# themattinthehatt/behavenet

Measured on AMD Instinct MI355X. Metric: AE training frames/sec (128x128x1, batch 256), higher is better.
Workload: dtype f32; 1 GPU; configs[1]: conv AE default arch, 1x128x128 f32 frames resident in HBM, 12 latents, batch 256 (chunks 200+56), fwd+bwd+Adam(amsgrad)

## Files before the change

### behavenet_amd/_hip.py

```python

import ctypes
import os

import torch

_LIB_NAME = 'libbehavenet_hip.so'
_LIB_PATH = os.environ.get('BN_HIP_LIB') or os.path.join(
    os.path.dirname(os.path.abspath(__file__)), _LIB_NAME)
_lib = None

ACT_NONE, ACT_LRELU, ACT_SIGMOID = 0, 1, 2

PROF_NONE, PROF_CONV_FWD, PROF_CONV_BWD_D, PROF_CONV_BWD_W = 0, 1, 2, 3
PROF_CONVT_FWD, PROF_CONVT_BWD_D, PROF_CONVT_BWD_W, PROF_ADAM = 4, 5, 6, 7
PROF_LINEAR_FWD, PROF_LINEAR_BWD = 8, 9

_c_int, _c_float, _c_size_t, _c_void_p = ctypes.c_int, ctypes.c_float, ctypes.c_size_t, ctypes.c_void_p

_CONV_GEOM = [_c_int] * 12
_ACT_WS = [_c_int, _c_float, _c_void_p, _c_size_t, _c_void_p]

OP_CONV_FWD, OP_CONV_BWD_D, OP_CONV_BWD_W = 1, 2, 3
OP_CONVT_FWD, OP_CONVT_BWD_D, OP_CONVT_BWD_W = 4, 5, 6

SIGNATURES = {
    'bn_version': (_c_int, []),
    'bn_build_arch': (ctypes.c_char_p, []),
    'bn_error_string': (ctypes.c_char_p, [_c_int]),
    'bn_set_force_generic': (_c_int, [_c_int]),
    'bn_set_bigk1_block_bytes': (_c_size_t, [_c_size_t]),
    'bn_conv_ws_bytes': (_c_size_t, [_c_int] + _CONV_GEOM),
    'bn_conv_taps_bytes': (_c_size_t, [_c_int] + _CONV_GEOM),
    'bn_conv_taps_pad': (_c_int, [_c_int, _c_void_p, _c_void_p, _c_void_p, _c_void_p]),
    'bn_conv2d_fwd': (_c_int, [_c_void_p] * 5 + _CONV_GEOM + _ACT_WS),
    'bn_conv2d_fwd_u8_ws_bytes': (_c_size_t, _CONV_GEOM + [_c_int]),
    'bn_conv2d_fwd_u8': (_c_int, [_c_void_p] * 4 + _CONV_GEOM + _ACT_WS),
    'bn_conv2d_bwd_data': (_c_int, [_c_void_p] * 5 + _CONV_GEOM + _ACT_WS),
    'bn_conv2d_bwd_weight': (
        _c_int, [_c_void_p] * 4 + _CONV_GEOM + [_c_int, _c_void_p, _c_size_t, _c_void_p]),
    'bn_convT2d_fwd': (_c_int, [_c_void_p] * 5 + _CONV_GEOM + _ACT_WS),
    'bn_convT2d_bwd_data': (_c_int, [_c_void_p] * 5 + _CONV_GEOM + _ACT_WS),
    'bn_convT2d_bwd_weight': (
        _c_int, [_c_void_p] * 4 + _CONV_GEOM + [_c_int, _c_void_p, _c_size_t, _c_void_p]),
    'bn_batchnorm_ws_bytes': (_c_size_t, [_c_int, _c_int]),
    'bn_batchnorm_stats': (_c_int, [_c_void_p] * 3 + [_c_int] * 3 + [_c_void_p, _c_size_t, _c_void_p]),
    'bn_batchnorm_finalize': (_c_int, [_c_void_p] * 5 + [_c_int] + [_c_float] * 3 + [_c_void_p]),
    'bn_batchnorm_act_fwd': (_c_int, [_c_void_p] * 6 + [_c_int] * 4 + [_c_float, _c_void_p]),
    'bn_batchnorm_train_fwd_chunks': (
        _c_int, [_c_void_p] * 11 + [_c_int] * 3 + [_c_float, _c_int, _c_float, _c_void_p, _c_size_t,
                                                  _c_void_p]),
    'bn_batchnorm_act_bwd_chunks': (
        _c_int, [_c_void_p] * 10 + [_c_int, _c_void_p] + [_c_int] * 4 + [_c_float, _c_void_p, _c_size_t,
                                                                        _c_void_p]),
    'bn_batchnorm_act_bwd': (
        _c_int, [_c_void_p] * 9 + [_c_int] * 6 + [_c_float, _c_void_p, _c_size_t, _c_void_p]),
    'bn_batchnorm_moment': (_c_int, [_c_void_p] * 3 + [_c_int] * 3 + [_c_void_p, _c_size_t, _c_void_p]),
    'bn_batchnorm_bwd_reduce': (
        _c_int, [_c_void_p] * 7 + [_c_int] * 4 + [_c_float, _c_void_p, _c_size_t, _c_void_p]),
    'bn_batchnorm_bwd_apply': (
        _c_int, [_c_void_p] * 9 + [_c_int] * 3 + [_c_float, _c_int, _c_float, _c_void_p]),
    'bn_maxpool2d_fwd': (_c_int, [_c_void_p] * 3 + [_c_int] * 9 + [_c_void_p]),
    'bn_maxpool2d_bwd': (_c_int, [_c_void_p] * 3 + [_c_int] * 9 + [_c_void_p]),
    'bn_maxpool2d_act_fwd': (_c_int, [_c_void_p] * 3 + [_c_int] * 4 + [ctypes.c_float, _c_void_p]),
    'bn_conv2d_pool2_act_fwd': (_c_int, [_c_void_p] * 5 + _CONV_GEOM + [_c_int, _c_float, _c_void_p]),
    'bn_conv2d_pool2_act_ok': (_c_int, _CONV_GEOM),
    'bn_conv2d_pool2_bwd_weight_ws_bytes': (_c_size_t, _CONV_GEOM),
# ... 237 lines not shown
    _check(load().bn_convT2d_fwd(
        _ptr(x, 'x'), _ptr(w, 'w'), _ptr(w5, 'w5', allow_none=True), _ptr(b, 'b', allow_none=True), _ptr(y, 'y'),
        *geom, act, slope, ws, nb, _stream()), 'bn_convT2d_fwd')
    return y


def convT2d_bwd_data(dy, w, geom, dact_src, dact, slope, w5=None):
    N, Ci, Hi, Wi = geom[:4]
    dx = torch.empty((N, Ci, Hi, Wi), dtype=torch.float32, device=dy.device)
    ws, nb = _workspace(OP_CONVT_BWD_D, geom, dy.device)
    _check(load().bn_convT2d_bwd_data(
        _ptr(dy, 'dy'), _ptr(w, 'w'), _ptr(w5, 'w5', allow_none=True), _ptr(dx, 'dx'),
        _ptr(dact_src, 'dact_src', allow_none=True), *geom, dact, slope, ws, nb, _stream()), 'bn_convT2d_bwd_data')
    return dx


def convT2d_bwd_weight(x, dy, dw, db, geom, accumulate):
    ws, nb = _workspace(OP_CONVT_BWD_W, geom, x.device)
    _check(lib_call('bn_convT2d_bwd_weight')(
        _ptr(x, 'x'), _ptr(dy, 'dy'), _ptr(dw, 'dw'), _ptr(db, 'db', allow_none=True), *geom,
        int(accumulate), ws, nb, _stream()), 'bn_convT2d_bwd_weight')


def conv2d_bf16_ok(geom, first=False):
    lib = load()
    return bool((lib.bn_conv2d_first_bf16_ok if first else lib.bn_conv2d_bf16_ok)(*[int(v) for v in geom]))


def conv_pack_w_bf16_bytes(w_shape):
    K, C, R, S = [int(v) for v in w_shape]
    return int(load().bn_conv_pack_w_bf16_bytes(K, C, R, S))


def conv_pack_w_bf16(w, out):
    K, C, R, S = w.shape
    if out.numel() * out.element_size() < conv_pack_w_bf16_bytes(w.shape):
        raise HipLibraryError('conv_pack_w_bf16: output buffer too small')
    _check(load().bn_conv_pack_w_bf16(_ptr(w, 'w'), out.data_ptr(), K, C, R, S, _stream()),
           'bn_conv_pack_w_bf16')
    return out


def _bf16_out(out, shape, dtype, device, what):
    if out is None:
        return torch.empty(shape, dtype=dtype, device=device)
    if tuple(out.shape) != tuple(shape) or out.dtype != dtype:
# ... 730 lines not shown
```

### behavenet_amd/csrc/bn_fast.h

```cpp
#pragma once
#include "bn_common.h"

struct BnFastPlan {
    bool supported;
    const char* kernel_name;
    size_t ws_bytes;
    int variant;
    int a, b, c, d;
};

BnFastPlan bn_fast_down_plan(const BnGeom& g);
BnFastPlan bn_fast_up_plan(const BnGeom& g);
BnFastPlan bn_fast_wgrad_plan(const BnGeom& g);

int bn_launch_down_fast(const BnFastPlan& plan, const float* big, const float* w,
                        const float* bias, float* out, const float* dact_src, const BnGeom& g,
                        int act, int dact, float slope, void* ws, hipStream_t st);
int bn_launch_up_fast(const BnFastPlan& plan, const float* small, const float* w,
                      const float* bias, float* out, const float* dact_src, const BnGeom& g,
                      int act, int dact, float slope, void* ws, hipStream_t st);
int bn_launch_wgrad_fast(const BnFastPlan& plan, const float* small, const float* big, float* dw,
                         const BnGeom& g, int accumulate, void* ws, hipStream_t st,
                         float* db = nullptr, int bias_side = 0, bool* bias_done = nullptr);

bool bn_wgrad_pool_c1_ok(const BnGeom& g);
size_t bn_wgrad_pool_c1_ws_bytes(const BnGeom& g);
int bn_launch_wgrad_pool_c1(const float* x, const float* dy, const float* y, const int* idx, float* dw, float* db,
                            const BnGeom& g, int act, float slope, int accumulate, void* ws, hipStream_t st);
bool bn_s1in1_pool_ok(const BnGeom& g);
int bn_launch_s1in1_pool(const float* big, const float* w, const float* bias, float* y, int* idx, const BnGeom& g,
                         int act, float slope, hipStream_t st);
bool bn_down2_pool_ok(const BnGeom& g);
int bn_launch_down2_pool(const float* big, const float* w, const float* bias, float* y, int* idx, const BnGeom& g,
                         int act, float slope, hipStream_t st);
bool bn_down2_supported(const BnGeom& g, int MR, int NR);
bool bn_down2_m16_supported(const BnGeom& g, int NR);
int bn_down2_splits(const BnGeom& g, int MR, int NR);
float bn_down2_fill(const BnGeom& g, int MR, int NR);
int bn_launch_down2(int MR, int NR, const float* big, const float* w, const float* bias,
                    float* out, const float* dact_src, const BnGeom& g, int act, int dact,
                    float slope, hipStream_t st, int splits = 1, void* ws = nullptr);

BnFastPlan bn_wgrad4_plan(const BnGeom& g);
int bn_launch_wgrad4(const BnFastPlan& plan, const float* small, const float* big, float* dw,
                     const BnGeom& g, int accumulate, void* ws, hipStream_t st, float* db,
                     int bias_side, bool* bias_done);

BnFastPlan bn_s5_up_plan(const BnGeom& g);
BnFastPlan bn_s5_wgrad_plan(const BnGeom& g);
int bn_launch_up_s5(const float* small, const float* w, const float* bias, float* out,
                    const float* dact_src, const BnGeom& g, int act, int dact, float slope,
                    hipStream_t st);
int bn_launch_wgrad_s5(const float* small, const float* big, float* dw, const BnGeom& g,
                       int accumulate, hipStream_t st);

BnFastPlan bn_edge_wgrad_plan(const BnGeom& g);
int bn_launch_edge_wgrad(const BnFastPlan& plan, const float* small, const float* big, float* dw,
                         const BnGeom& g, int accumulate, void* ws, hipStream_t st,
                         float* db = nullptr, int bias_side = 0, bool* bias_done = nullptr);
bool bn_s1c1_ok(const BnGeom& g);
int bn_launch_s1c1(const float* big, const float* w, const float* bias, float* out, const float* dact_src,
                   const BnGeom& g, int act, int dact, float slope, hipStream_t st);
bool bn_s1in1_ok(const BnGeom& g);
int bn_launch_s1in1(const float* big, const float* w, const float* bias, float* out, const float* dact_src,
                    const BnGeom& g, int act, int dact, float slope, hipStream_t st);
BnFastPlan bn_edge_down_plan(const BnGeom& g);
const char* bn_edge_down_kernel_name(const BnGeom& g, int act, bool has_dact, bool u8);
const char* bn_edge_up_kernel_name(const BnGeom& g, bool loss);
int bn_launch_edge_down(const float* big, const float* w, const float* bias, float* out,
// ... 43 lines not shown
```

### behavenet_amd/csrc/capi.hip

```cpp
#include <math.h>
#include <stdio.h>
#include <stdlib.h>
#include <string.h>
#include <hip/hip_ext.h>
#include "bn_common.h"
#include "bn_launch.h"
#include "bn_fast.h"

namespace {
struct ProfState {
    int family = BN_PROF_NONE;
    int C = 0, K = 0;
    static const int kMaxSlots = 2048;
    hipEvent_t ev[4 * kMaxSlots];
    bool taken[kMaxSlots], bracketed[kMaxSlots];
    int created = 0;
    int used = 0;
    double total_ms = 0.0, main_ms = 0.0;
    long launches = 0, main_launches = 0;
    bool bracket = true;
    int nth = -1, seen = 0;
    char kernel_name[96] = "";
} g_prof;

// ... 1246 lines not shown
    const BnGeom g = convT_geom(N, Ci, Hi, Wi, Co, R, S, stride, crop_t, crop_l, Ho, Wo);
    if (!bn_geom_ok(g)) return BN_E_BADARG;
    return run_down(BN_PROF_CONVT_BWD_D, dy, w, w5, nullptr, dx, dact_src, g, BN_ACT_NONE, dact, slope,
                    ws, ws_bytes, (hipStream_t)stream);
}

extern "C" int bn_convT2d_bwd_weight(const float* x, const float* dy, float* dw, float* db, int N,
                                     int Ci, int Hi, int Wi, int Co, int R, int S, int stride,
                                     int crop_t, int crop_l, int Ho, int Wo, int accumulate,
                                     void* ws, size_t ws_bytes, bn_stream_t stream) {
    if (!x || !dy || !dw) return BN_E_BADARG;
    const BnGeom g = convT_geom(N, Ci, Hi, Wi, Co, R, S, stride, crop_t, crop_l, Ho, Wo);
    if (!bn_geom_ok(g)) return BN_E_BADARG;
    hipStream_t st = (hipStream_t)stream;
    bool bias_done = false;
    int rc = run_wgrad(BN_PROF_CONVT_BWD_W, x, dy, dw, g, accumulate, ws, ws_bytes, st, db, 2,
                       &bias_done);
    if (rc) return rc;
    if (db && !bias_done)
        rc = bn_launch_channel_sum(dy, db, N, Co, Ho * Wo, accumulate, ws, ws_bytes, st);
    return rc;
}

extern "C" int bn_act_fwd(const float* x, float* y, size_t n, int act, float slope,
                          bn_stream_t stream) {
    if (!x || !y || n == 0) return BN_E_BADARG;
    return bn_launch_act_fwd(x, y, n, act, slope, (hipStream_t)stream);
}

extern "C" int bn_act_bwd(const float* dy, const float* y, float* dpre, size_t n, int act,
                          float slope, bn_stream_t stream) {
    if (!dy || !y || !dpre) return BN_E_BADARG;
    if (n == 0) return 0;
    return bn_launch_act_bwd(dy, y, dpre, n, act, slope, (hipStream_t)stream);
}

extern "C" size_t bn_batchnorm_ws_bytes(int N, int C) {
    return (N > 0 && C > 0) ? bn_batchnorm_ws_bytes_impl(N, C) : 0;
}

extern "C" int bn_batchnorm_stats(const float* x, float* mean, float* var, int N, int C, int HW,
                                  void* ws, size_t ws_bytes, bn_stream_t stream) {
    if (!x || !mean || !var || N <= 0 || C <= 0 || HW <= 0) return BN_E_BADARG;
    if (!ws || ws_bytes < bn_batchnorm_ws_bytes_impl(N, C)) return BN_E_WORKSPACE;
    return bn_launch_bn_stats(x, mean, var, N, C, HW, ws, (hipStream_t)stream);
}
// ... 498 lines not shown
```

### behavenet_amd/csrc/conv_mfma_wgrad4.hip

```cpp
#include <stdlib.h>
#include "bn_common.h"
#include "bn_fast.h"
#include "bn_reduce.h"

typedef float floatx4 __attribute__((ext_vector_type(4)));
typedef float floatx2 __attribute__((ext_vector_type(2)));

#define W4_STR2(x) #x
#define W4_STR(x) W4_STR2(x)
#ifndef W4_LOOP_SHIFT
#define W4_LOOP_SHIFT 0
#endif
#define W4_THREADS 512
#define W4_TA 64
#define W4_TB 32
#define W4_TPX 64
#define W4_X0 4
#define W4_SLICES 8
#define W4_MAX_LDS (160 * 1024)
#define W4_OOB 0x7fffffff

static inline int ilog2_exact_w4(int v) {
    int l = 0;
    while ((1 << l) < v) ++l;
// ... 155 lines not shown
    }
}

template <int Q_, int ST_ = 2, int PTH_ = 0>
struct W4S {
    static constexpr int Q = Q_, ST = ST_, PT_H = PTH_ ? PTH_ : W4_TPX / Q, IH = ST * (PT_H - 1) + 5;
    static constexpr int KS = PT_H * Q / 4;
    static constexpr int RW = ST * Q + 8, C4 = RW / 4;
    static constexpr int ROWG = IH * C4;
    static constexpr int GPB = (ROWG & 1) ? ROWG : ROWG + 1;
    static constexpr int BCH = 4 * GPB;
    static constexpr int BIGG = W4_TB * GPB;
    static constexpr int SMALLW = W4_TA * W4_TPX;
    static constexpr int BUFW = SMALLW + 4 * ((BIGG + 63) / 64 * 64);
    static constexpr int NBIG = (BIGG + W4_THREADS - 1) / W4_THREADS;
    static constexpr int NSM = SMALLW / 4 / W4_THREADS;
};

__device__ __forceinline__ void w4_dma16(__amdgpu_buffer_rsrc_t rsrc, float* lds, int voffset,
                                         int soffset) {
    __builtin_amdgcn_raw_ptr_buffer_load_lds(rsrc, lds, 16, voffset, soffset, 0, 0);
}

template <int QQ, int BIAS, bool GEN, int KV, int ST = 2, int PTH = 0, bool CW = false, int NA = 4, int NB = 2>
__global__ __launch_bounds__(W4_THREADS, 1) void k_wgrad4s_mfma(
    const float* __restrict__ small, const float* __restrict__ big, float* __restrict__ part,
    float* __restrict__ bias_part, BnGeom g, int n_stages, int splits, int lg_tpf, int nbias, int ncb) {
    extern __shared__ __attribute__((aligned(16))) float smem[];
    using T = W4S<QQ, ST, PTH>;
    static_assert(ST == 2 || GEN, "stride 1: the general row limits");
    static_assert(!CW || (GEN && ST == 2 && (QQ & 3) == 0), "column windows: general stride-2 stages");
    constexpr int Q = T::Q, RW = T::RW, BUFW = T::BUFW;
    constexpr bool HALF = (Q & 3) == 2;
    static_assert(((Q & 3) == 0 || (HALF && ST == 2 && GEN && (T::PT_H & 1) == 0)) && T::KS >= 1 && T::KS <= 16,
                  "stage geometry");
    const int tid = threadIdx.x, lane = tid & 63;
    const int wv = __builtin_amdgcn_readfirstlane(tid >> 6);
    constexpr int NG = 8 / (NA * NB), KSG = T::KS / NG;
    static_assert(NA * NB * NG == 8 && KSG * NG == T::KS && KSG >= 1 && NG <= 4, "wave groups");
    static_assert(NG == 1 || (!HALF && !CW && (KSG & (KSG - 1)) == 0 &&
                              ((4 * KSG) % Q == 0 || Q % (4 * KSG) == 0)), "wave groups: whole rows or parts of one");
    const int blk = wv % (NA * NB), grp = wv / (NA * NB);
    const int ablk = NG == 1 ? wv >> 1 : blk / NB, bblk = NG == 1 ? wv & 1 : blk % NB;
    const int lj = lane & 15, kk = lane >> 4;

    const int n_btiles = (g.Cb + W4_TB - 1) / W4_TB;
    const int atile = blockIdx.x / n_btiles, btile = blockIdx.x - atile * n_btiles;
    const int a0 = atile * W4_TA, b0 = btile * W4_TB;
    const int PQ = g.Hs * g.Ws, HWb = g.Hb * g.Wb;

    floatx4 acc[25];
#pragma unroll
    for (int tp = 0; tp < 25; ++tp) acc[tp] = (floatx4){0.f, 0.f, 0.f, 0.f};
    float bsum = 0.f;

    const __amdgpu_buffer_rsrc_t rs_small = __builtin_amdgcn_make_buffer_rsrc(
        (void*)small, 0, (int)((size_t)g.N * g.Cs * PQ * 4), 0x00020000);
    const int pt_rows = ST == 2 ? 1 : g.pt;
    const int lead = pt_rows * g.Wb + (CW ? W4_X0 : 0);
    const __amdgpu_buffer_rsrc_t rs_big = __builtin_amdgcn_make_buffer_rsrc(
        (void*)(big - lead), 0, (int)(((size_t)g.N * g.Cb * HWb + lead) * 4), 0x00020000);
    int soff[T::NSM], srow = 0;
#pragma unroll
    for (int j = 0; j < T::NSM; ++j) {
        const int e = tid + W4_THREADS * j;
        const int a = e >> 4;
        const int pix0 = 4 * ((e & 15) ^ (a & 15));
        const int spix = CW ? (pix0 / Q) * g.Ws + (pix0 - (pix0 / Q) * Q) : pix0;
        soff[j] = (a0 + a < g.Cs && pix0 < 4 * T::KS) ? ((a0 + a) * PQ + spix) * 4 : W4_OOB;
        srow |= (pix0 / Q) << (8 * j);
// ... 117 lines not shown
                    }
                } else if (NG == 1) {
                    if (r == 3 && sx == 4 && ks < NDMA) {
                        if (more) issue_dma(ks, nbuf, n0n, p0n);
                    }
                } else if (sx == 4 && r < NG && ks * NG + r < NDMA) {
                    if (more) issue_dma(ks * NG + r, nbuf, n0n, p0n);
                }
                __builtin_amdgcn_sched_barrier(0);
            }
        }
    };

    const int tpf_mask = (1 << lg_tpf) - 1;
    const int tpf_gen = (g.Hs + T::PT_H - 1) / T::PT_H;
    auto frame_of = [&](const int s) __attribute__((always_inline)) {
        if constexpr (GEN) return lg_tpf == 0 ? s : (int)__umulhi((unsigned)s, (unsigned)lg_tpf);
        else return s >> lg_tpf;
    };
    auto row_of = [&](const int s, const int f) __attribute__((always_inline)) {
        if constexpr (GEN) return (s - f * tpf_gen) * T::PT_H;
        else return (s & tpf_mask) * T::PT_H;
    };
    int st = blockIdx.y;
    if (st < n_stages) {
        const int f0 = frame_of(st);
#pragma unroll
        for (int d = 0; d < NDMA; ++d) issue_dma(d, 0, f0, row_of(st, f0));
    }
    int ab_cur = abase[0], ab_oth = abase[1], bb_cur = bbase[0], bb_oth = bbase[1];
    int cur = 0;
#ifdef W4_LOOP_ALIGN
    asm volatile(".p2align " W4_STR(W4_LOOP_ALIGN) "\n .rept " W4_STR(W4_LOOP_SHIFT) "\n s_nop 0\n .endr" ::: "memory");
#endif
    for (; st < n_stages; st += splits) {
        asm volatile("s_waitcnt vmcnt(0)" ::: "memory");
        __syncthreads();
        const int nx = st + splits;
        const int fx = frame_of(nx);
        stage_body(ab_cur, bb_cur, bsp_cur, cur ^ 1, nx < n_stages, fx, row_of(nx, fx));
        cur ^= 1;
        int tmp = ab_cur; ab_cur = ab_oth; ab_oth = tmp;
        tmp = bb_cur; bb_cur = bb_oth; bb_oth = tmp;
        if (HALF) { tmp = bsp_cur; bsp_cur = bsp_oth; bsp_oth = tmp; }
    }

    if (BIAS != 0) {
        bsum += __shfl_xor(bsum, 16, 64);
        bsum += __shfl_xor(bsum, 32, 64);
        float* bdst = bias_part + ((size_t)blockIdx.y * NG + grp) * nbias;
        if (BIAS == 1 && btile == 0 && bblk == 0 && kk == 0) {
            const int a = a0 + ablk * 16 + lj;
            if (a < g.Cs) bdst[a] = bsum;
        }
        if (BIAS == 2 && atile == 0 && ablk == 0 && kk == 0) {
            const int bb = b0 + bblk * 16 + lj;
            if (bb < g.Cb) bdst[bb] = bsum;
        }
    }

    float* dst = part + ((size_t)blockIdx.y * NG + grp) * 25 * g.Cs * g.Cb;
    const int b = b0 + bblk * 16 + lj;
    if (b < g.Cb) {
#pragma unroll
        for (int tp = 0; tp < 25; ++tp) {
#pragma unroll
            for (int e = 0; e < 4; ++e) {
                const int a = a0 + ablk * 16 + 4 * kk + e;
                if (a < g.Cs) dst[((size_t)tp * g.Cs + a) * g.Cb + b] = acc[tp][e];
            }
        }
    }
}

static bool wgrad4_tile(const BnGeom& g, Wgrad4Tile* t, size_t* lds_bytes) {
    const int lgQ = ilog2_exact_w4(g.Ws), lgP = ilog2_exact_w4(g.Hs);
    if (lgQ < 2 || lgQ > 5 || lgP < 0) return false;
    if (g.pt != 1 || g.pl != 1) return false;
    if ((g.Wb & 3) != 0 || g.Wb < 2 * g.Ws) return false;
    const int PQ = g.Hs * g.Ws;
    if (PQ >= W4_TPX) {
        t->F = 1;
        t->PT_H = W4_TPX / g.Ws;
    } else {
        t->F = W4_TPX / PQ;
        t->PT_H = g.Hs;
    }
    t->lgPTQ = ilog2_exact_w4(t->PT_H * g.Ws);
    t->tiles_per_frame = (t->F == 1) ? g.Hs / t->PT_H : 1;
    t->n_stages = ((g.N + t->F - 1) / t->F) * t->tiles_per_frame;
    t->IH = 2 * (t->PT_H - 1) + 5;
    const int RW = 2 * g.Ws + 8;
    t->FSb = t->IH * RW;
    t->rows_per_b = t->F * t->IH;
    t->row_groups = t->rows_per_b * (RW / 4);
// ... 306 lines not shown
                                                    t.n_stages, t.splits, lg_tpf, t.nbias);
        W4S_CASE(3, 0) W4S_CASE(3, 1) W4S_CASE(3, 2) W4S_CASE(4, 0) W4S_CASE(4, 1) W4S_CASE(4, 2)
        W4S_CASE(5, 0) W4S_CASE(5, 1) W4S_CASE(5, 2)
#undef W4S_CASE
        }
    } else
    switch (ilog2_exact_w4(g.Ws)) {
        case 2: rc = launch_wgrad4<2>(grid, lds, st, small, big, (float*)ws, bias_part, g, t); break;
        case 3: rc = launch_wgrad4<3>(grid, lds, st, small, big, (float*)ws, bias_part, g, t); break;
        case 4: rc = launch_wgrad4<4>(grid, lds, st, small, big, (float*)ws, bias_part, g, t); break;
        case 5: rc = launch_wgrad4<5>(grid, lds, st, small, big, (float*)ws, bias_part, g, t); break;
        default: break;
    }
    if (rc) return rc;
    if (fuse) {
        rc = bn_launch_sum_partials_pair((const float*)ws, dw, 25 * g.Cs * g.Cb, g.Cs * g.Cb, 25,
                                         bias_part, db, t.nbias, t.splits, accumulate, st);
        if (bias_done) *bias_done = true;
        return rc;
    }
    return bn_launch_sum_partials((const float*)ws, dw, 25 * g.Cs * g.Cb, t.splits, accumulate,
                                  g.Cs * g.Cb, 25, st);
}
```

### behavenet_amd/hip_functions.py

```python

import collections.abc
import contextlib
import os
import threading
import warnings

import torch

from behavenet_amd import _hip

LRELU_SLOPE = 0.05

_direct_grads = False


class accumulate_into_param_grads(object):

    def __enter__(self):
        global _direct_grads
        self._prev = _direct_grads
        _direct_grads = True

    def __exit__(self, *exc):
        global _direct_grads
# ... 43 lines not shown
    o = _ones_cache.get(key)
    if o is None:
        o = torch.ones_like(t.detach())
        _ones_cache[key] = o
    return o


def backward_chunks(chunk_losses, streams=None, single_pass=False):
    global _single_pass, _use_side_stream
    _single_pass = bool(single_pass and len(chunk_losses) == 1)
    saved_side = _use_side_stream
    if _single_pass:
        _use_side_stream = False
    try:
        with accumulate_into_param_grads():
            for i, loss in enumerate(chunk_losses):
                stream = streams[i] if streams is not None and i < len(streams) else None
                seed = _ones_like(loss) if loss.dim() > 0 else None
                if stream is not None:
                    with torch.cuda.stream(stream):
                        loss.backward(seed)
                else:
                    loss.backward(seed)
    finally:
        _single_pass = False
        _use_side_stream = saved_side


_capturing = False


def capturing():
    return _capturing


class DeferredLoss(object):

    def __init__(self, tensors, fn, reduce_over_ranks=False):
        self.tensors, self.fn = tensors, fn
        self.reduce_over_ranks = bool(reduce_over_ranks)


class LazyLoss(collections.abc.Mapping):

    def __init__(self, readbacks, fn):
        self._rbs, self._fn, self._dict = readbacks, fn, None

    def resolve(self):
        if self._dict is None:
# ... 303 lines not shown
    taps = getattr(ctx, 'taps', None)
    for i in range(n_layers - 1, -1, -1):
        layer = plan[i]
        g = layer.geom(n)
        w = weights[i]
        x_in = acts[i]
        if x_in.dtype == torch.uint8:
            x_in = _hip.u8_to_unit_float(x_in) \
                if ctx.needs_input_grad[first_param + 2 * i] else None
        need_w = ctx.needs_input_grad[first_param + 2 * i]
        need_b = ctx.needs_input_grad[first_param + 1 + 2 * i]
        if need_w:
            gw = _grad_buffer(ctx.param_refs[2 * i])
            gb = _grad_buffer(ctx.param_refs[2 * i + 1]) if need_b else None
            direct = gw is not None and (gb is not None or not need_b)
            if direct:
                dw, db = gw, gb
            else:
                dw = torch.empty_like(w)
                db = torch.empty((layer.cout,), dtype=w.dtype, device=w.device) if need_b \
                    else None
            wgrad = _hip.conv2d_bwd_weight if layer.kind == 'conv' else _hip.convT2d_bwd_weight
            side = _side_stream(w.device) if (direct and _use_side_stream) else None
            if side is not None:
                main = torch.cuda.current_stream(w.device)
                ev = torch.cuda.Event()
                ev.record(main)
                with torch.cuda.stream(side):
                    side.wait_event(ev)
                    wgrad(x_in, dpre, dw, db, g, True)
                dpre.record_stream(side)
                x_in.record_stream(side)
                _report_ready(ctx.param_refs[2 * i:2 * i + 2])
            else:
                wgrad(x_in, dpre, dw, db, g, direct)
                if direct:
                    _report_ready(ctx.param_refs[2 * i:2 * i + 2])
            if not direct:
                grads[2 * i], grads[2 * i + 1] = dw, db
        if i > 0 or ctx.need_dx:
            dact_src = acts[i] if i > 0 else None
            dact = plan[i - 1].act if i > 0 else _hip.ACT_NONE
            w5 = taps[i] if taps else None
            if layer.kind == 'conv':
                dpre = _hip.conv2d_bwd_data(dpre, w, g, dact_src, dact, LRELU_SLOPE, w5=w5)
            else:
                dpre = _hip.convT2d_bwd_data(dpre, w, g, dact_src, dact, LRELU_SLOPE, w5=w5)
# ... 1035 lines not shown
```

### include/behavenet_hip.h

```cpp
#ifndef BEHAVENET_HIP_H
#define BEHAVENET_HIP_H

#include <stddef.h>

#ifdef __cplusplus
extern "C" {
#endif

#define BN_E_BADARG   (-1)
#define BN_E_SHAPE    (-2)
#define BN_E_WORKSPACE (-3)

#define BN_ACT_NONE    0
#define BN_ACT_LRELU   1
#define BN_ACT_SIGMOID 2

typedef void* bn_stream_t;

int         bn_version(void);
const char* bn_build_arch(void);
const char* bn_error_string(int code);

#define BN_OP_CONV_FWD    1
#define BN_OP_CONV_BWD_D  2
// ... 18 lines not shown
                       int N, int C, int H, int W, int K, int R, int S, int stride,
                       int pad_t, int pad_l, int P, int Q,
                       int dact, float slope, void* ws, size_t ws_bytes, bn_stream_t stream);

int bn_conv2d_bwd_weight(const float* x, const float* dy, float* dw, float* db,
                         int N, int C, int H, int W, int K, int R, int S, int stride,
                         int pad_t, int pad_l, int P, int Q,
                         int accumulate, void* ws, size_t ws_bytes, bn_stream_t stream);

int bn_convT2d_fwd(const float* x, const float* w, const float* w5, const float* b, float* y,
                   int N, int Ci, int Hi, int Wi, int Co, int R, int S, int stride,
                   int crop_t, int crop_l, int Ho, int Wo,
                   int act, float slope, void* ws, size_t ws_bytes, bn_stream_t stream);

int bn_convT2d_bwd_data(const float* dy, const float* w, const float* w5, float* dx, const float* dact_src,
                        int N, int Ci, int Hi, int Wi, int Co, int R, int S, int stride,
                        int crop_t, int crop_l, int Ho, int Wo,
                        int dact, float slope, void* ws, size_t ws_bytes, bn_stream_t stream);

int bn_convT2d_bwd_weight(const float* x, const float* dy, float* dw, float* db,
                          int N, int Ci, int Hi, int Wi, int Co, int R, int S, int stride,
                          int crop_t, int crop_l, int Ho, int Wo,
                          int accumulate, void* ws, size_t ws_bytes, bn_stream_t stream);

int bn_act_fwd(const float* x, float* y, size_t n, int act, float slope, bn_stream_t stream);
int bn_act_bwd(const float* dy, const float* y, float* dpre, size_t n,
               int act, float slope, bn_stream_t stream);

int bn_maxpool2d_fwd(const float* x, float* y, int* idx, int planes, int H, int W, int Ho, int Wo,
                     int k, int stride, int pad_t, int pad_l, bn_stream_t stream);
int bn_maxpool2d_bwd(const float* dy, const int* idx, float* dx, int planes, int H, int W,
                     int Ho, int Wo, int k, int stride, int pad_t, int pad_l, bn_stream_t stream);
int bn_conv2d_pool2_act_fwd(const float* x, const float* w, const float* b, float* y, int* idx,
                            int N, int C, int H, int W, int K, int R, int S, int stride,
                            int pad_t, int pad_l, int P, int Q, int act, float slope, bn_stream_t stream);
int bn_conv2d_pool2_act_ok(int N, int C, int H, int W, int K, int R, int S, int stride,
                           int pad_t, int pad_l, int P, int Q);
size_t bn_conv2d_pool2_bwd_weight_ws_bytes(int N, int C, int H, int W, int K, int R, int S, int stride,
                                           int pad_t, int pad_l, int P, int Q);
int bn_conv2d_pool2_bwd_weight(const float* x, const float* dy, const float* y, const int* idx, float* dw, float* db,
                               int N, int C, int H, int W, int K, int R, int S, int stride,
                               int pad_t, int pad_l, int P, int Q, int act, float slope, int accumulate,
                               void* ws, size_t ws_bytes, bn_stream_t stream);
int bn_maxpool2d_act_fwd(const float* x, float* y, int* idx, int planes, int H, int W, int act, float slope,
                         bn_stream_t stream);
int bn_maxpool2d_act_bwd(const float* dy, const float* y, const int* idx, float* dx, int planes, int H, int W,
// ... 188 lines not shown
```

Measured before the change: 58860 frames/s.

## Batch several small-layer weight-gradient convolutions into one persistent stream-K style launch

Weight-gradient work for eligible stride-2 5x5 layers is queued during the single-pass backward instead of being launched per layer. Up to eight such layers then run in one kernel that splits their tile×stage work evenly across all compute units into per-tile partial slabs, followed by one combine kernel that reduces the slabs into dw/db. This targets per-layer launch overhead and poor CU fill for small layers. The cost is extra workspace and a second reduction pass, and the gradients are now produced later, which delays when the parameters are reported ready for the optimizer.

```diff
diff --git a/behavenet_amd/_hip.py b/behavenet_amd/_hip.py
--- a/behavenet_amd/_hip.py
+++ b/behavenet_amd/_hip.py
@@ -42,6 +42,11 @@
     'bn_convT2d_bwd_data': (_c_int, [_c_void_p] * 5 + _CONV_GEOM + _ACT_WS),
     'bn_convT2d_bwd_weight': (
         _c_int, [_c_void_p] * 4 + _CONV_GEOM + [_c_int, _c_void_p, _c_size_t, _c_void_p]),
+    'bn_wgrad_jobs_ok': (_c_int, [_c_int] + _CONV_GEOM),
+    'bn_wgrad_jobs_ws_bytes': (_c_size_t, [_c_int, _c_void_p, _c_int]),
+    'bn_wgrad_jobs_plan': (_c_int, [_c_int, _c_void_p, _c_int, _c_void_p, _c_int]),
+    'bn_wgrad_jobs': (
+        _c_int, [_c_int] + [_c_void_p] * 6 + [_c_void_p, _c_size_t, _c_int, _c_void_p]),
     'bn_batchnorm_ws_bytes': (_c_size_t, [_c_int, _c_int]),
     'bn_batchnorm_stats': (_c_int, [_c_void_p] * 3 + [_c_int] * 3 + [_c_void_p, _c_size_t, _c_void_p]),
     'bn_batchnorm_finalize': (_c_int, [_c_void_p] * 5 + [_c_int] + [_c_float] * 3 + [_c_void_p]),
@@ -325,6 +330,61 @@
         int(accumulate), ws, nb, _stream()), 'bn_convT2d_bwd_weight')
 
 
+WGRAD_JOBS_MAX = 8
+_jobs_ok = {}
+
+
+def wgrad_jobs_ok(op, geom):
+    key = (_generic_epoch, op) + tuple(geom)
+    v = _jobs_ok.get(key)
+    if v is None:
+        v = _jobs_ok[key] = bool(load().bn_wgrad_jobs_ok(op, *[int(q) for q in geom]))
+    return v
+
+
+def _jobs_geoms(jobs):
+    flat = []
+    for op, geom in jobs:
+        flat.append(int(op))
+        flat.extend(int(v) for v in geom)
+    return (ctypes.c_int * (13 * len(jobs)))(*flat)
+
+
+def wgrad_jobs_ws_bytes(jobs, n_wg=0):
+    return int(load().bn_wgrad_jobs_ws_bytes(len(jobs), _jobs_geoms(jobs), int(n_wg)))
+
+
+def wgrad_jobs_plan(jobs, n_wg):
+    lib, geoms = load(), _jobs_geoms(jobs)
+    n = lib.bn_wgrad_jobs_plan(len(jobs), geoms, int(n_wg), None, 0)
+    _check(min(n, 0), 'bn_wgrad_jobs_plan')
+    segs = (ctypes.c_int * (6 * max(n, 1)))()
+    _check(min(lib.bn_wgrad_jobs_plan(len(jobs), geoms, int(n_wg), segs, n), 0), 'bn_wgrad_jobs_plan')
+    return [tuple(segs[6 * i:6 * i + 6]) for i in range(n)]
+
+
+def wgrad_jobs(jobs, n_wg=0, ws=None):
+    n = len(jobs)
+    if n == 0:
+        return
+    geoms = _jobs_geoms([(j[0], j[1]) for j in jobs])
+    lib = load()
+    if ws is None:
+        nbytes = int(lib.bn_wgrad_jobs_ws_bytes(n, geoms, int(n_wg)))
+        if nbytes == 0:
+            raise HipLibraryError('wgrad_jobs: a layer that bn_wgrad_jobs does not serve')
+        wsp = _arena(jobs[0][2].device, nbytes, 'wgrad_jobs')
+    else:
+        wsp, nbytes = ws.data_ptr(), ws.numel()
+    vp = ctypes.c_void_p * n
+    xp = vp(*[_ptr(j[2], 'x') for j in jobs])
+    dyp = vp(*[_ptr(j[3], 'dy') for j in jobs])
+    dwp = vp(*[_ptr(j[4], 'dw') for j in jobs])
+    dbp = vp(*[_ptr(j[5], 'db', allow_none=True) for j in jobs])
+    acc = (ctypes.c_int * n)(*[int(bool(j[6])) for j in jobs])
+    _check(lib.bn_wgrad_jobs(n, geoms, xp, dyp, dwp, dbp, acc, wsp, nbytes, int(n_wg), _stream()), 'bn_wgrad_jobs')
+
+
 def conv2d_bf16_ok(geom, first=False):
     lib = load()
     return bool((lib.bn_conv2d_first_bf16_ok if first else lib.bn_conv2d_bf16_ok)(*[int(v) for v in geom]))
diff --git a/behavenet_amd/csrc/bn_fast.h b/behavenet_amd/csrc/bn_fast.h
--- a/behavenet_amd/csrc/bn_fast.h
+++ b/behavenet_amd/csrc/bn_fast.h
@@ -45,6 +45,15 @@
 int bn_launch_wgrad4(const BnFastPlan& plan, const float* small, const float* big, float* dw,
                      const BnGeom& g, int accumulate, void* ws, hipStream_t st, float* db,
                      int bias_side, bool* bias_done);
+
+#define BN_WGRAD_JOBS_MAX 8
+#define BN_WGRAD_JOBS_MAX_TILES 16
+bool bn_wgrad4_jobs_geom_ok(const BnGeom& g, int bias_side);
+size_t bn_wgrad4_jobs_ws_bytes(int n_jobs, const BnGeom* gs, const int* bias, int n_wg);
+int bn_wgrad4_jobs_plan(int n_jobs, const BnGeom* gs, const int* bias, int n_wg, int* segs, int max_segs);
+int bn_launch_wgrad4_jobs(int n_jobs, const BnGeom* gs, const int* bias, const float* const* small,
+                          const float* const* big, float* const* dw, float* const* db, const int* accumulate,
+                          void* ws, size_t ws_bytes, int n_wg, hipStream_t st);
 
 BnFastPlan bn_s5_up_plan(const BnGeom& g);
 BnFastPlan bn_s5_wgrad_plan(const BnGeom& g);
diff --git a/behavenet_amd/csrc/capi.hip b/behavenet_amd/csrc/capi.hip
--- a/behavenet_amd/csrc/capi.hip
+++ b/behavenet_amd/csrc/capi.hip
@@ -1292,6 +1292,95 @@
     return rc;
 }
 
+static bool wgrad_jobs_route(const BnGeom& g, int bias_side) {
+    if (force_generic()) return false;
+    BnGeom g5;
+    BigK bk;
+    BigK1 b1;
+    if (taps_plan(2, g, &g5) || bigk_plan(2, g, &g5, &bk) || bigk1_plan(2, g, &g5, &b1) || chan_plan(2, g, &g5))
+        return false;
+    if (bn_qg2_wgrad_supported(g) || bn_qgemm_supported(g) || bn_s5win_supported(g) || s5_wgrad_by_col(g)) return false;
+    if (bn_s5_wgrad_plan(g).supported || bn_edge_wgrad_plan(g).supported) return false;
+    const BnFastPlan plan = bn_fast_wgrad_plan(g);
+    return plan.supported && plan.variant == 4 && bn_wgrad4_jobs_geom_ok(g, bias_side);
+}
+static bool wgrad_jobs_geom(const int* q, BnGeom* g, int* side) {
+    if (q[0] == BN_OP_CONV_BWD_W) {
+        *g = conv_geom(q[1], q[2], q[3], q[4], q[5], q[6], q[7], q[8], q[9], q[10], q[11], q[12]);
+        *side = 1;
+    } else if (q[0] == BN_OP_CONVT_BWD_W) {
+        *g = convT_geom(q[1], q[2], q[3], q[4], q[5], q[6], q[7], q[8], q[9], q[10], q[11], q[12]);
+        *side = 2;
+    } else return false;
+    return bn_geom_ok(*g);
+}
+static int wgrad_jobs_n_wg(int n_wg) {
+    if (n_wg > 0) return n_wg;
+    static int cus = 0;
+    if (cus == 0) {
+        int dev = 0, v = 0;
+        if (hipGetDevice(&dev) != hipSuccess ||
+            hipDeviceGetAttribute(&v, hipDeviceAttributeMultiprocessorCount, dev) != hipSuccess || v <= 0) {
+            (void)hipGetLastError();
+            return 256;
+        }
+        cus = v;
+    }
+    return cus;
+}
+
+extern "C" int bn_wgrad_jobs_ok(int op, int N, int C, int H, int W, int K, int R, int S, int stride, int off_t,
+                                int off_l, int P, int Q) {
+    const int q[13] = {op, N, C, H, W, K, R, S, stride, off_t, off_l, P, Q};
+    BnGeom g;
+    int side = 0;
+    if (!wgrad_jobs_geom(q, &g, &side)) return 0;
+    return wgrad_jobs_route(g, side) ? 1 : 0;
+}
+
+extern "C" size_t bn_wgrad_jobs_ws_bytes(int n_jobs, const int* geoms, int n_wg) {
+    if (n_jobs < 1 || n_jobs > BN_WGRAD_JOBS_MAX || !geoms || n_wg < 0) return 0;
+    BnGeom gs[BN_WGRAD_JOBS_MAX];
+    int bias[BN_WGRAD_JOBS_MAX];
+    for (int j = 0; j < n_jobs; ++j) {
+        if (!wgrad_jobs_geom(geoms + 13 * j, &gs[j], &bias[j]) || !wgrad_jobs_route(gs[j], bias[j])) return 0;
+    }
+    return bn_wgrad4_jobs_ws_bytes(n_jobs, gs, bias, wgrad_jobs_n_wg(n_wg));
+}
+
+extern "C" int bn_wgrad_jobs_plan(int n_jobs, const int* geoms, int n_wg, int* segs, int max_segs) {
+    if (n_jobs < 1 || n_jobs > BN_WGRAD_JOBS_MAX || !geoms || n_wg < 1 || max_segs < 0) return BN_E_BADARG;
+    BnGeom gs[BN_WGRAD_JOBS_MAX];
+    int bias[BN_WGRAD_JOBS_MAX];
+    for (int j = 0; j < n_jobs; ++j) {
+        if (!wgrad_jobs_geom(geoms + 13 * j, &gs[j], &bias[j])) return BN_E_BADARG;
+        if (!wgrad_jobs_route(gs[j], bias[j])) return BN_E_SHAPE;
+    }
+    return bn_wgrad4_jobs_plan(n_jobs, gs, bias, n_wg, segs, max_segs);
+}
+
+extern "C" int bn_wgrad_jobs(int n_jobs, const int* geoms, const float* const* x, const float* const* dy,
+                             float* const* dw, float* const* db, const int* accumulate, void* ws, size_t ws_bytes,
+                             int n_wg, bn_stream_t stream) {
+    if (n_jobs < 1 || n_jobs > BN_WGRAD_JOBS_MAX || !geoms || !x || !dy || !dw || !db || !accumulate || n_wg < 0)
+        return BN_E_BADARG;
+    BnGeom gs[BN_WGRAD_JOBS_MAX];
+    int bias[BN_WGRAD_JOBS_MAX];
+    const float* small[BN_WGRAD_JOBS_MAX];
+    const float* big[BN_WGRAD_JOBS_MAX];
+    for (int j = 0; j < n_jobs; ++j) {
+        int side = 0;
+        if (!x[j] || !dy[j] || !dw[j]) return BN_E_BADARG;
+        if (!wgrad_jobs_geom(geoms + 13 * j, &gs[j], &side)) return BN_E_BADARG;
+        if (!wgrad_jobs_route(gs[j], side)) return BN_E_SHAPE;
+        small[j] = side == 1 ? dy[j] : x[j];
+        big[j] = side == 1 ? x[j] : dy[j];
+        bias[j] = db[j] ? side : 0;
+    }
+    return bn_launch_wgrad4_jobs(n_jobs, gs, bias, small, big, dw, db, accumulate, ws, ws_bytes,
+                                 wgrad_jobs_n_wg(n_wg), (hipStream_t)stream);
+}
+
 extern "C" int bn_act_fwd(const float* x, float* y, size_t n, int act, float slope,
                           bn_stream_t stream) {
     if (!x || !y || n == 0) return BN_E_BADARG;
diff --git a/behavenet_amd/csrc/conv_mfma_wgrad4.hip b/behavenet_amd/csrc/conv_mfma_wgrad4.hip
--- a/behavenet_amd/csrc/conv_mfma_wgrad4.hip
+++ b/behavenet_amd/csrc/conv_mfma_wgrad4.hip
@@ -1,4 +1,5 @@
 #include <stdlib.h>
+#include <string.h>
 #include "bn_common.h"
 #include "bn_fast.h"
 #include "bn_reduce.h"
@@ -201,10 +202,12 @@
     __builtin_amdgcn_raw_ptr_buffer_load_lds(rsrc, lds, 16, voffset, soffset, 0, 0);
 }
 
-template <int QQ, int BIAS, bool GEN, int KV, int ST = 2, int PTH = 0, bool CW = false, int NA = 4, int NB = 2>
-__global__ __launch_bounds__(W4_THREADS, 1) void k_wgrad4s_mfma(
+template <int QQ, int BIAS, bool GEN, int KV, int ST = 2, int PTH = 0, bool CW = false, int NA = 4, int NB = 2,
+          bool LOCAL = false>
+__device__ __forceinline__ void w4s_body(
     const float* __restrict__ small, const float* __restrict__ big, float* __restrict__ part,
-    float* __restrict__ bias_part, BnGeom g, int n_stages, int splits, int lg_tpf, int nbias, int ncb) {
+    float* __restrict__ bias_part, const BnGeom& g, const int tile, const int st0, const int n_stages,
+    const int splits, int lg_tpf, int nbias, int ncb) {
     extern __shared__ __attribute__((aligned(16))) float smem[];
     using T = W4S<QQ, ST, PTH>;
     static_assert(ST == 2 || GEN, "stride 1: the general row limits");
@@ -224,7 +227,7 @@
     const int lj = lane & 15, kk = lane >> 4;
 
     const int n_btiles = (g.Cb + W4_TB - 1) / W4_TB;
-    const int atile = blockIdx.x / n_btiles, btile = blockIdx.x - atile * n_btiles;
+    const int atile = tile / n_btiles, btile = tile - atile * n_btiles;
     const int a0 = atile * W4_TA, b0 = btile * W4_TB;
     const int PQ = g.Hs * g.Ws, HWb = g.Hb * g.Wb;
 
@@ -388,7 +391,7 @@
         if constexpr (GEN) return (s - f * tpf_gen) * T::PT_H;
         else return (s & tpf_mask) * T::PT_H;
     };
-    int st = blockIdx.y;
+    int st = st0;
     if (st < n_stages) {
         const int f0 = frame_of(st);
 #pragma unroll
@@ -414,18 +417,19 @@
     if (BIAS != 0) {
         bsum += __shfl_xor(bsum, 16, 64);
         bsum += __shfl_xor(bsum, 32, 64);
-        float* bdst = bias_part + ((size_t)blockIdx.y * NG + grp) * nbias;
+        float* bdst = bias_part + (size_t)grp * nbias;
         if (BIAS == 1 && btile == 0 && bblk == 0 && kk == 0) {
             const int a = a0 + ablk * 16 + lj;
-            if (a < g.Cs) bdst[a] = bsum;
+            if (a < g.Cs) bdst[LOCAL ? a - a0 : a] = bsum;
         }
         if (BIAS == 2 && atile == 0 && ablk == 0 && kk == 0) {
             const int bb = b0 + bblk * 16 + lj;
-            if (bb < g.Cb) bdst[bb] = bsum;
-        }
-    }
-
-    float* dst = part + ((size_t)blockIdx.y * NG + grp) * 25 * g.Cs * g.Cb;
+            if (bb < g.Cb) bdst[LOCAL ? bb - b0 : bb] = bsum;
+        }
+    }
+
+    static_assert(!LOCAL || NG == 1, "tile-local slabs: whole-tile instantiations");
+    float* dst = part + (size_t)grp * 25 * g.Cs * g.Cb;
     const int b = b0 + bblk * 16 + lj;
     if (b < g.Cb) {
 #pragma unroll
@@ -433,10 +437,23 @@
 #pragma unroll
             for (int e = 0; e < 4; ++e) {
                 const int a = a0 + ablk * 16 + 4 * kk + e;
-                if (a < g.Cs) dst[((size_t)tp * g.Cs + a) * g.Cb + b] = acc[tp][e];
+                if (a < g.Cs) {
+                    if (LOCAL) dst[(tp * W4_TA + (a - a0)) * W4_TB + (b - b0)] = acc[tp][e];
+                    else dst[((size_t)tp * g.Cs + a) * g.Cb + b] = acc[tp][e];
+                }
             }
         }
     }
+}
+
+template <int QQ, int BIAS, bool GEN, int KV, int ST = 2, int PTH = 0, bool CW = false, int NA = 4, int NB = 2>
+__global__ __launch_bounds__(W4_THREADS, 1) void k_wgrad4s_mfma(
+    const float* __restrict__ small, const float* __restrict__ big, float* __restrict__ part,
+    float* __restrict__ bias_part, BnGeom g, int n_stages, int splits, int lg_tpf, int nbias, int ncb) {
+    constexpr int NG = 8 / (NA * NB);
+    w4s_body<QQ, BIAS, GEN, KV, ST, PTH, CW, NA, NB, false>(
+        small, big, part + (size_t)blockIdx.y * NG * 25 * g.Cs * g.Cb, bias_part + (size_t)blockIdx.y * NG * nbias, g,
+        (int)blockIdx.x, (int)blockIdx.y, n_stages, splits, lg_tpf, nbias, ncb);
 }
 
 static bool wgrad4_tile(const BnGeom& g, Wgrad4Tile* t, size_t* lds_bytes) {
@@ -789,3 +806,270 @@
     return bn_launch_sum_partials((const float*)ws, dw, 25 * g.Cs * g.Cb, t.splits, accumulate,
                                   g.Cs * g.Cb, 25, st);
 }
+
+#define W4J_TILE_FLOATS (25 * W4_TA * W4_TB)
+#define W4J_SLAB_FLOATS (W4J_TILE_FLOATS + W4_TA)
+#define W4J_MAX_WG 4096
+#define W4J_MAX_PAIRS (BN_WGRAD_JOBS_MAX * BN_WGRAD_JOBS_MAX_TILES)
+
+struct W4Job {
+    const float* small;
+    const float* big;
+    BnGeom g;
+    int n_stages, lg_tpf;
+    int bias;
+    int tiles, inst;
+    int u0, pair0;
+};
+struct W4Jobs {
+    W4Job job[BN_WGRAD_JOBS_MAX];
+    int n_jobs, n_wg, U;
+    float* ws;
+    unsigned short slab0[W4J_MAX_PAIRS + 1];
+    unsigned short wg0[W4J_MAX_PAIRS];
+};
+struct W4CombineJob {
+    float* dw;
+    float* db;
+    int Cs, Cb, bias, accumulate, tiles, pair0;
+};
+struct W4Combine {
+    W4CombineJob job[BN_WGRAD_JOBS_MAX];
+    int n_jobs;
+    const float* ws;
+    unsigned short slab0[W4J_MAX_PAIRS + 1];
+};
+
+static inline __host__ __device__ unsigned w4j_lo(unsigned b, unsigned U, unsigned n) {
+    return (unsigned)(((unsigned long long)b * U) / n);
+}
+static inline unsigned w4j_owner(unsigned u, unsigned U, unsigned n) {
+    return (unsigned)((((unsigned long long)u + 1) * n - 1) / U);
+}
+
+__global__ __launch_bounds__(W4_THREADS, 1) void k_wgrad4s_jobs(W4Jobs p) {
+    const unsigned b = blockIdx.x;
+    if ((int)b >= p.n_wg) return;
+    const unsigned lo = w4j_lo(b, p.U, p.n_wg), hi = w4j_lo(b + 1, p.U, p.n_wg);
+    int j = 0;
+    while (j + 1 < p.n_jobs && lo >= (unsigned)p.job[j + 1].u0) ++j;
+    int tile = (int)(lo - (unsigned)p.job[j].u0) / p.job[j].n_stages;
+    int s0 = (int)(lo - (unsigned)p.job[j].u0) - tile * p.job[j].n_stages;
+    const int pair = p.job[j].pair0 + tile;
+    int slab = (int)p.slab0[pair] + ((int)b - (int)p.wg0[pair]);
+    bool first = true;
+    for (unsigned u = lo; u < hi;) {
+        const int n_stages = p.job[j].n_stages;
+        const int left = (int)(hi - u);
+        const int s1 = n_stages - s0 < left ? n_stages : s0 + left;
+        if (!first) {
+            asm volatile("s_waitcnt vmcnt(0)" ::: "memory");
+            __syncthreads();
+        }
+        first = false;
+        const BnGeom g = p.job[j].g;
+        const float* small = p.job[j].small;
+        const float* big = p.job[j].big;
+        const int lg_tpf = p.job[j].lg_tpf;
+        float* sl = p.ws + (size_t)slab * W4J_SLAB_FLOATS;
+        float* bsl = sl + W4J_TILE_FLOATS;
+#define W4J_CASE(L, B)                                                                                     \
+    case 3 * (L - 3) + B:                                                                                  \
+        w4s_body<(1 << L), B, false, 5, 2, 0, false, 4, 2, true>(small, big, sl, bsl, g, tile, s0, s1, 1, lg_tpf, 0, 1); \
+        break;
+        switch (p.job[j].inst) {
+            W4J_CASE(3, 0) W4J_CASE(3, 1) W4J_CASE(3, 2)
+            W4J_CASE(4, 0) W4J_CASE(4, 1) W4J_CASE(4, 2)
+            W4J_CASE(5, 0) W4J_CASE(5, 1) W4J_CASE(5, 2)
+            default: break;
+        }
+#undef W4J_CASE
+        u += (unsigned)(s1 - s0);
+        ++slab;
+        s0 = 0;
+        if (s1 == n_stages && ++tile == p.job[j].tiles) { tile = 0; ++j; }
+    }
+}
+
+#define W4C_BLOCKS (W4J_TILE_FLOATS / 4 / 64)
+__global__ __launch_bounds__(256) void k_wgrad_jobs_combine(W4Combine p) {
+    __shared__ floatx4 red[4][64];
+    const int pair = blockIdx.y;
+    int j = 0;
+    while (j + 1 < p.n_jobs && pair >= p.job[j + 1].pair0) ++j;
+    const W4CombineJob& jb = p.job[j];
+    const int tile = pair - jb.pair0;
+    const int n_btiles = (jb.Cb + W4_TB - 1) / W4_TB;
+    const int atile = tile / n_btiles, btile = tile - atile * n_btiles;
+    const int a0 = atile * W4_TA, b0 = btile * W4_TB;
+    const int z0 = p.slab0[pair], z1 = p.slab0[pair + 1];
+    const int il = threadIdx.x & 63, zl = threadIdx.x >> 6;
+    const bool bias_row = blockIdx.x == W4C_BLOCKS;
+    const bool bias_mine = jb.db && ((jb.bias == 1 && btile == 0 && a0 + il < jb.Cs) ||
+                                     (jb.bias == 2 && atile == 0 && il < W4_TB && b0 + il < jb.Cb));
+    const int e = bias_row ? W4J_TILE_FLOATS + il : (blockIdx.x * 64 + il) * 4;
+    const int tap = e / (W4_TA * W4_TB), a = (e / W4_TB) % W4_TA, bl = e % W4_TB;
+    const bool live = bias_row ? bias_mine : (a0 + a < jb.Cs && b0 + bl < jb.Cb);
+    floatx4 s0 = {0.f, 0.f, 0.f, 0.f}, s1 = s0, s2 = s0, s3 = s0;
+    if (live) {
+        const float* src = p.ws + (size_t)(z0 + zl) * W4J_SLAB_FLOATS + e;
+        const size_t zs = (size_t)4 * W4J_SLAB_FLOATS;
+        int z = z0 + zl;
+        if (bias_row) {
+            for (; z + 12 < z1; z += 16, src += 4 * zs) {
+                s0.x += src[0]; s1.x += src[zs]; s2.x += src[2 * zs]; s3.x += src[3 * zs];
+            }
+            for (; z < z1; z += 4, src += zs) s0.x += src[0];
+        } else {
+            for (; z + 12 < z1; z += 16, src += 4 * zs) {
+                s0 += *reinterpret_cast<const floatx4*>(src);
+                s1 += *reinterpret_cast<const floatx4*>(src + zs);
+                s2 += *reinterpret_cast<const floatx4*>(src + 2 * zs);
+                s3 += *reinterpret_cast<const floatx4*>(src + 3 * zs);
+            }
+            for (; z < z1; z += 4, src += zs) s0 += *reinterpret_cast<const floatx4*>(src);
+        }
+    }
+    red[zl][il] = (s0 + s1) + (s2 + s3);
+    __syncthreads();
+    if (zl != 0 || !live) return;
+    const floatx4 v = (red[0][il] + red[1][il]) + (red[2][il] + red[3][il]);
+    if (bias_row) {
+        float* o = jb.db + (jb.bias == 1 ? a0 : b0) + il;
+        *o = jb.accumulate ? *o + v.x : v.x;
+        return;
+    }
+    float* o = jb.dw + ((size_t)(a0 + a) * jb.Cb + b0 + bl) * 25 + tap;
+#pragma unroll
+    for (int k = 0; k < 4; ++k)
+        if (b0 + bl + k < jb.Cb) o[25 * k] = jb.accumulate ? o[25 * k] + v[k] : v[k];
+}
+
+bool bn_wgrad4_jobs_geom_ok(const BnGeom& g, int bias_side) {
+    if (g.R != 5 || g.S != 5 || g.stride != 2 || g.KV != 0 || g.K0 != 0 || g.CsS != 0) return false;
+    if (g.Cs < 16 || g.Cb < 16) return false;
+    Wgrad4Tile t;
+    size_t lds = 0;
+    if (!wgrad4_tile(g, &t, &lds) || !wgrad4s_ok(g, t)) return false;
+    int na, nb;
+    if (w4g1_groups(g, &na, &nb) != 1) return false;
+    if (bias_side == 2 && (g.Hb > 2 * g.Hs || g.Wb > 2 * g.Ws)) return false;
+    const int tiles = ((g.Cs + W4_TA - 1) / W4_TA) * ((g.Cb + W4_TB - 1) / W4_TB);
+    return tiles <= BN_WGRAD_JOBS_MAX_TILES;
+}
+
+static int w4j_build(int n_jobs, const BnGeom* gs, const int* bias, int n_wg, W4Jobs* p) {
+    if (n_jobs < 1 || n_jobs > BN_WGRAD_JOBS_MAX || n_wg < 1 || n_wg > W4J_MAX_WG) return BN_E_BADARG;
+    memset(p, 0, sizeof(*p));
+    unsigned long long U = 0;
+    int pairs = 0;
+    for (int j = 0; j < n_jobs; ++j) {
+        const BnGeom& g = gs[j];
+        if (bias[j] < 0 || bias[j] > 2 || !bn_wgrad4_jobs_geom_ok(g, bias[j])) return BN_E_SHAPE;
+        Wgrad4Tile t;
+        size_t lds = 0;
+        wgrad4_tile(g, &t, &lds);
+        W4Job& jb = p->job[j];
+        jb.g = g;
+        jb.n_stages = t.n_stages;
+        jb.lg_tpf = ilog2_exact_w4(t.tiles_per_frame);
+        jb.bias = bias[j];
+        jb.tiles = ((g.Cs + W4_TA - 1) / W4_TA) * ((g.Cb + W4_TB - 1) / W4_TB);
+        jb.inst = 3 * (ilog2_exact_w4(g.Ws) - 3) + bias[j];
+        jb.u0 = (int)U;
+        jb.pair0 = pairs;
+        U += (unsigned long long)jb.tiles * jb.n_stages;
+        pairs += jb.tiles;
+        if (U >= 0x7fffffffull) return BN_E_SHAPE;
+    }
+    p->n_jobs = n_jobs;
+    p->U = (int)U;
+    p->n_wg = (unsigned long long)n_wg < U ? n_wg : (int)U;
+    int pr = 0;
+    for (int j = 0; j < n_jobs; ++j)
+        for (int t = 0; t < p->job[j].tiles; ++t, ++pr) {
+            const unsigned f = (unsigned)p->job[j].u0 + (unsigned)t * p->job[j].n_stages;
+            const unsigned w0 = w4j_owner(f, p->U, p->n_wg), w1 = w4j_owner(f + p->job[j].n_stages - 1, p->U, p->n_wg);
+            p->wg0[pr] = (unsigned short)w0;
+            p->slab0[pr + 1] = (unsigned short)(p->slab0[pr] + (w1 - w0 + 1));
+        }
+    return 0;
+}
+
+size_t bn_wgrad4_jobs_ws_bytes(int n_jobs, const BnGeom* gs, const int* bias, int n_wg) {
+    W4Jobs p;
+    if (w4j_build(n_jobs, gs, bias, n_wg, &p)) return 0;
+    return (size_t)p.slab0[p.job[n_jobs - 1].pair0 + p.job[n_jobs - 1].tiles] * W4J_SLAB_FLOATS * sizeof(float);
+}
+
+int bn_wgrad4_jobs_plan(int n_jobs, const BnGeom* gs, const int* bias, int n_wg, int* segs, int max_segs) {
+    W4Jobs p;
+    const int rc = w4j_build(n_jobs, gs, bias, n_wg, &p);
+    if (rc) return rc;
+    int n = 0;
+    for (unsigned b = 0; b < (unsigned)p.n_wg; ++b) {
+        const unsigned lo = w4j_lo(b, p.U, p.n_wg), hi = w4j_lo(b + 1, p.U, p.n_wg);
+        int j = 0;
+        while (j + 1 < p.n_jobs && lo >= (unsigned)p.job[j + 1].u0) ++j;
+        int tile = (int)(lo - (unsigned)p.job[j].u0) / p.job[j].n_stages;
+        int s0 = (int)(lo - (unsigned)p.job[j].u0) - tile * p.job[j].n_stages;
+        const int pair = p.job[j].pair0 + tile;
+        int slab = (int)p.slab0[pair] + ((int)b - (int)p.wg0[pair]);
+        for (unsigned u = lo; u < hi;) {
+            const int n_stages = p.job[j].n_stages;
+            const int left = (int)(hi - u);
+            const int s1 = n_stages - s0 < left ? n_stages : s0 + left;
+            if (segs && n < max_segs) {
+                int* s = segs + 6 * (size_t)n;
+                s[0] = (int)b; s[1] = j; s[2] = tile; s[3] = s0; s[4] = s1; s[5] = slab;
+            }
+            ++n;
+            u += (unsigned)(s1 - s0);
+            ++slab;
+            s0 = 0;
+            if (s1 == n_stages && ++tile == p.job[j].tiles) { tile = 0; ++j; }
+        }
+    }
+    return n;
+}
+
+int bn_launch_wgrad4_jobs(int n_jobs, const BnGeom* gs, const int* bias, const float* const* small,
+                          const float* const* big, float* const* dw, float* const* db, const int* accumulate,
+                          void* ws, size_t ws_bytes, int n_wg, hipStream_t st) {
+    W4Jobs p;
+    int rc = w4j_build(n_jobs, gs, bias, n_wg, &p);
+    if (rc) return rc;
+    const int pairs = p.job[n_jobs - 1].pair0 + p.job[n_jobs - 1].tiles;
+    const size_t need = (size_t)p.slab0[pairs] * W4J_SLAB_FLOATS * sizeof(float);
+    if (!ws || ws_bytes < need || ((uintptr_t)ws & 15)) return BN_E_WORKSPACE;
+    W4Combine c;
+    memset(&c, 0, sizeof(c));
+    size_t lds = 0;
+    for (int j = 0; j < n_jobs; ++j) {
+        if (!small[j] || !big[j] || !dw[j] || (bias[j] && !db[j])) return BN_E_BADARG;
+        if (((uintptr_t)small[j] | (uintptr_t)big[j]) & 15) return BN_E_BADARG;
+        p.job[j].small = small[j];
+        p.job[j].big = big[j];
+        c.job[j] = {dw[j], bias[j] ? db[j] : nullptr, gs[j].Cs, gs[j].Cb, bias[j], accumulate[j], p.job[j].tiles,
+                    p.job[j].pair0};
+        const int lgq = ilog2_exact_w4(gs[j].Ws);
+        const size_t l = (size_t)2 * 4 * (lgq == 3 ? W4S<8>::BUFW : lgq == 4 ? W4S<16>::BUFW : W4S<32>::BUFW);
+        lds = l > lds ? l : lds;
+    }
+    p.ws = (float*)ws;
+    c.n_jobs = n_jobs;
+    c.ws = (const float*)ws;
+    memcpy(c.slab0, p.slab0, sizeof(c.slab0));
+    static bool attr_set = false;
+    if (!attr_set) {
+        hipError_t e = hipFuncSetAttribute((const void*)k_wgrad4s_jobs, hipFuncAttributeMaxDynamicSharedMemorySize,
+                                           W4_MAX_LDS);
+        if (e != hipSuccess) return (int)e;
+        attr_set = true;
+    }
+    hipLaunchKernelGGL(k_wgrad4s_jobs, dim3(p.n_wg), dim3(W4_THREADS), lds, st, p);
+    BN_LAUNCH_CHECK();
+    hipLaunchKernelGGL(k_wgrad_jobs_combine, dim3(W4C_BLOCKS + 1, pairs), dim3(256), 0, st, c);
+    BN_LAUNCH_CHECK();
+    return 0;
+}
diff --git a/behavenet_amd/hip_functions.py b/behavenet_amd/hip_functions.py
--- a/behavenet_amd/hip_functions.py
+++ b/behavenet_amd/hip_functions.py
@@ -89,9 +89,31 @@
                         loss.backward(seed)
                 else:
                     loss.backward(seed)
+            _flush_wgrad_jobs()
     finally:
+        del _wgrad_jobs[:]
         _single_pass = False
         _use_side_stream = saved_side
+
+
+_use_wgrad_jobs = os.environ.get('BN_WGRAD_JOBS', '1') != '0'
+_wgrad_jobs = []
+
+
+def _queue_wgrad_job(job, params):
+    _wgrad_jobs.append((job, params))
+    if len(_wgrad_jobs) >= _hip.WGRAD_JOBS_MAX:
+        _flush_wgrad_jobs()
+
+
+def _flush_wgrad_jobs():
+    if not _wgrad_jobs:
+        return
+    queued = list(_wgrad_jobs)
+    del _wgrad_jobs[:]
+    _hip.wgrad_jobs([job for job, _ in queued])
+    for _, params in queued:
+        _report_ready(params)
 
 
 _capturing = False
@@ -441,7 +463,10 @@
                     else None
             wgrad = _hip.conv2d_bwd_weight if layer.kind == 'conv' else _hip.convT2d_bwd_weight
             side = _side_stream(w.device) if (direct and _use_side_stream) else None
-            if side is not None:
+            op = _hip.OP_CONV_BWD_W if layer.kind == 'conv' else _hip.OP_CONVT_BWD_W
+            if _use_wgrad_jobs and _single_pass and direct and _hip.wgrad_jobs_ok(op, g):
+                _queue_wgrad_job((op, g, x_in, dpre, dw, db, True), ctx.param_refs[2 * i:2 * i + 2])
+            elif side is not None:
                 main = torch.cuda.current_stream(w.device)
                 ev = torch.cuda.Event()
                 ev.record(main)
diff --git a/include/behavenet_hip.h b/include/behavenet_hip.h
--- a/include/behavenet_hip.h
+++ b/include/behavenet_hip.h
@@ -64,6 +64,14 @@
                           int N, int Ci, int Hi, int Wi, int Co, int R, int S, int stride,
                           int crop_t, int crop_l, int Ho, int Wo,
                           int accumulate, void* ws, size_t ws_bytes, bn_stream_t stream);
+
+int bn_wgrad_jobs_ok(int op, int N, int C, int H, int W, int K, int R, int S, int stride,
+                     int off_t, int off_l, int P, int Q);
+size_t bn_wgrad_jobs_ws_bytes(int n_jobs, const int* geoms, int n_wg);
+int bn_wgrad_jobs_plan(int n_jobs, const int* geoms, int n_wg, int* segs, int max_segs);
+int bn_wgrad_jobs(int n_jobs, const int* geoms, const float* const* x, const float* const* dy,
+                  float* const* dw, float* const* db, const int* accumulate,
+                  void* ws, size_t ws_bytes, int n_wg, bn_stream_t stream);
 
 int bn_act_fwd(const float* x, float* y, size_t n, int act, float slope, bn_stream_t stream);
 int bn_act_bwd(const float* dy, const float* y, float* dpre, size_t n,
```

Result: no change. 58970 frames/s (median of 6 runs) (+0.2%).
